# lukasino1214/soc_real_time_renderer

Hardware: AMD Instinct MI355X
Metric: frames/sec + ms/pass, Sponza 3840x2160 deferred+SSAO+TAA (higher is better)
Workload: dtype f32 (fp16/unorm8/d32 storage)

## Files before the change

include/soc_rt.h:

```cpp
#ifndef SOC_RT_H
#define SOC_RT_H

#include <stdint.h>
#include <stddef.h>

#ifdef __cplusplus
extern "C" {
#endif

#define SOC_RT_ABI_VERSION 1

#define SOC_OK 0
#define SOC_E_INVALID_ARG (-1)
#define SOC_E_SHAPE (-2)
#define SOC_E_HIP (-3)
#define SOC_E_UNSUPPORTED (-4)

struct ihipStream_t;
typedef struct ihipStream_t* soc_stream;

typedef enum soc_format {
    SOC_FMT_RGBA16F = 1,
    SOC_FMT_D32F = 2,
    SOC_FMT_R8_UNORM = 3,
// ... 240 lines not shown
#define SOC_PHASE_ALL 3

#define SOC_RENDERER_TIMING 1
#define SOC_RENDERER_UNFUSED_BLOOM 2
#define SOC_RENDERER_SERIAL 4
#define SOC_RENDERER_UNFUSED_TONEMAP 8
#define SOC_RENDERER_FUSED_HISTOGRAM 16
#define SOC_RENDERER_EXACT_BLOOM 32
#define SOC_RENDERER_UNFUSED_HISTOGRAM 64
#define SOC_RENDERER_NO_SKY_SPLIT 128
#define SOC_RENDERER_STATIC_INPUTS 256
#define SOC_RENDERER_VELOCITY_SLOTS 512
#define SOC_RENDERER_BLOOM_IN_COMPOSITION 1024
#define SOC_RENDERER_SKY_LANE_HIGH 2048
#define SOC_RENDERER_SKY_LANE_PROBE 4096

soc_renderer* soc_renderer_create(const soc_frame_images* images, uint32_t flags);
void soc_renderer_destroy(soc_renderer* r);
int soc_renderer_execute(soc_renderer* r, const soc_globals* g, int32_t phase, soc_stream stream);
int soc_renderer_set_exposure_pixels(soc_renderer* r, uint64_t total_pixels, int32_t wide_accumulator);
int32_t soc_renderer_pass_count(const soc_renderer* r);
const char* soc_renderer_pass_name(const soc_renderer* r, int32_t index);
const char* soc_renderer_pass_group(const soc_renderer* r, int32_t index);
float soc_renderer_pass_ms(soc_renderer* r, int32_t index);
#define SOC_RENDERER_TIMING_RING 256
int soc_renderer_set_pass_timing(soc_renderer* r, int32_t index, int32_t enable);
int soc_renderer_reset_timing(soc_renderer* r);
int soc_renderer_pass_stats(soc_renderer* r, int32_t index, float* total_ms, int32_t* frames);
int32_t soc_renderer_pass_event_times(soc_renderer* r, int32_t index, void* base, float* start_ms, float* end_ms,
                                      int32_t n);
int32_t soc_renderer_current_history(const soc_renderer* r);
int soc_renderer_set_current_history(soc_renderer* r, int32_t index);
int soc_renderer_set_async(soc_renderer* r, int32_t enable);
int32_t soc_renderer_side_queue(const soc_renderer* r);
int32_t soc_renderer_side_queue_probe_frames(const soc_renderer* r);

enum soc_resource {
    SOC_RES_ALBEDO = 0, SOC_RES_EMISSIVE, SOC_RES_NORMAL, SOC_RES_DEPTH, SOC_RES_VELOCITY,
    SOC_RES_SUN_SHADOW, SOC_RES_NOISE,
    SOC_RES_BLOOM_MIP0, SOC_RES_BLOOM_MIP1, SOC_RES_BLOOM_MIP2, SOC_RES_BLOOM_MIP3,
    SOC_RES_BLOOM_OUTPUT,
    SOC_RES_SSAO, SOC_RES_SSAO_BLUR, SOC_RES_CLOUDS, SOC_RES_COLOR,
    SOC_RES_PREVIOUS_COLOR, SOC_RES_RESOLVED,
    SOC_RES_PREVIOUS_VELOCITY,
    SOC_RES_AUTO_EXPOSURE,
    SOC_RES_OUTPUT,
    SOC_RES_VISIBILITY,
    SOC_RES_HISTOGRAM_PARTIALS,
    SOC_RES_SKY_COLOR,
    SOC_RES_SKY_HISTOGRAM_PARTIALS,
    SOC_RES_USER0 = 32,
    SOC_RES_COUNT = 64
};
#define SOC_PASS_MAX_USES 16
#define SOC_PASS_ASYNC 1
typedef struct soc_pass_desc {
    const char* name;
    const char* group;
    int32_t phase;
    uint32_t flags;
    int32_t read_count, write_count;
    int32_t reads[SOC_PASS_MAX_USES];
    int32_t writes[SOC_PASS_MAX_USES];
} soc_pass_desc;
typedef int32_t (*soc_pass_callback)(void* user, const soc_globals* g, const soc_frame_images* images, soc_stream stream);
int soc_renderer_add_pass(soc_renderer* r, const soc_pass_desc* desc, soc_pass_callback fn, void* user,
// ... 85 lines not shown
```

soc_real_time_renderer_amd/__init__.py:

```python
from __future__ import annotations

import ctypes as C
import os
from typing import Optional

import numpy as np
import torch

from . import _abi
from ._abi import (FMT_D32F, FMT_R8_UNORM, FMT_RGBA8_SRGB, FMT_RGBA8_UNORM, FMT_RGBA16F, FMT_RGBA32F,
                   PHASE_ALL, PHASE_POST_EXPOSURE, PHASE_PRE_EXPOSURE, AutoExposure, Camera, FrameImages, Globals,
                   SocImg)

PKG_DIR = os.path.dirname(os.path.abspath(__file__))
LIB_PATH = os.path.join(PKG_DIR, "lib", os.environ.get("SOC_RT_LIB_VARIANT", "libsoc_rt.so"))

__all__ = ["SocError", "lib", "img", "Globals", "Camera", "AutoExposure", "globals_defaults", "frame_update",
           "bloom_downsample", "bloom_upsample", "bloom_chain", "ssao_prepare_noise", "ssao_generation",
           "ssao_blur", "cloud_rendering", "composition", "generate_luminance_histogram",
           "resolve_luminance_histogram", "temporal_antialiasing", "copy_image", "tone_mapping", "upload_globals",
           "Renderer", "read_image", "write_png", "write_exr", "FMT_RGBA16F", "FMT_D32F", "FMT_R8_UNORM", "FMT_RGBA8_UNORM", "FMT_RGBA8_SRGB",
           "FMT_RGBA32F", "PHASE_PRE_EXPOSURE", "PHASE_POST_EXPOSURE", "PHASE_ALL"]


# ... 419 lines not shown
        _check(lib().soc_renderer_add_pass(self.handle, C.byref(d), cb, None, before.encode() if before else None),
               "soc_renderer_add_pass")
        self._callbacks = getattr(self, "_callbacks", []) + [cb]

    def pass_uses(self, index: int):
        rd, wr = C.c_uint64(0), C.c_uint64(0)
        _check(lib().soc_renderer_pass_uses(self.handle, index, C.byref(rd), C.byref(wr)), "soc_renderer_pass_uses")

        def names(m):
            return {(_abi.RESOURCES[b] if b < len(_abi.RESOURCES) else f"USER{b - _abi.RES_USER0}")
                    for b in range(_abi.RES_COUNT) if (m >> b) & 1}
        return names(rd.value), names(wr.value)

    def pass_dependencies(self, index: int):
        buf = (C.c_int32 * 64)()
        n = lib().soc_renderer_pass_dependencies(self.handle, index, buf, 64)
        if n < 0:
            _check(int(n), "soc_renderer_pass_dependencies")
        return [int(buf[i]) for i in range(min(n, 64))]

    def pass_carry_dependencies(self, index: int):
        buf = (C.c_int32 * 64)()
        n = lib().soc_renderer_pass_carry_dependencies(self.handle, index, buf, 64)
        if n < 0:
            _check(int(n), "soc_renderer_pass_carry_dependencies")
        return [int(buf[k]) for k in range(n)]

    def pass_lane(self, index: int) -> int:
        return int(lib().soc_renderer_pass_lane(self.handle, index))

    def set_async(self, enable: bool) -> None:
        _check(lib().soc_renderer_set_async(self.handle, int(bool(enable))), "soc_renderer_set_async")

    def current_history(self) -> int:
        return int(lib().soc_renderer_current_history(self.handle))

    def velocity_slot(self) -> int:
        return 1 - self.current_history()

    def resolved(self) -> torch.Tensor:
        return self.frame["history_color"][self.current_history()]

    STATE_VERSION = 1

    def save_state(self, path: Optional[str] = None) -> dict:
        torch.cuda.synchronize()
        h = self.current_history()
        st = {"version": np.int32(self.STATE_VERSION), "history_index": np.int32(h),
              "history_color": self.frame["history_color"][h].cpu().numpy(),
              "history_velocity": self.frame["history_velocity"][h].cpu().numpy(),
              "auto_exposure": self.frame["auto_exposure"].cpu().numpy()}
        if path:
            np.savez(path, **st)
        return st

    def load_state(self, state) -> None:
        st = dict(np.load(state, allow_pickle=False)) if isinstance(state, (str, os.PathLike)) else state
        if int(st["version"]) != self.STATE_VERSION:
            raise ValueError(f"load_state: checkpoint version {int(st['version'])}, expected {self.STATE_VERSION}")
        h = int(st["history_index"])
        if h not in (0, 1):
            raise ValueError(f"load_state: history_index {h} is not 0 or 1")
        srcs = {}
        for key in ("history_color", "history_velocity"):
            dst = self.frame[key][h]
            src = np.asarray(st[key])
# ... 24 lines not shown
```

soc_real_time_renderer_amd/_abi.py:

```python
from __future__ import annotations

import ctypes as C

SOC_OK = 0
SOC_E_INVALID_ARG = -1
SOC_E_SHAPE = -2
SOC_E_HIP = -3
SOC_E_UNSUPPORTED = -4

FMT_RGBA16F = 1
FMT_D32F = 2
FMT_R8_UNORM = 3
FMT_RGBA8_UNORM = 4
FMT_RGBA8_SRGB = 5
FMT_RGBA32F = 6

BYTES_PER_PIXEL = {FMT_RGBA16F: 8, FMT_D32F: 4, FMT_R8_UNORM: 1, FMT_RGBA8_UNORM: 4, FMT_RGBA8_SRGB: 4,
                   FMT_RGBA32F: 16}

MAX_POINT_LIGHTS = 128
MAX_SPOT_LIGHTS = 128
BIN_COUNT = 256
SSAO_MAX_KERNEL = 26

# ... 166 lines not shown
    "soc_mat4_ortho_rh_no": (None, [C.POINTER(C.c_float)] + [C.c_float] * 6),
    "soc_mat4_look_at_rh": (None, [C.POINTER(C.c_float)] * 4),
    "soc_mat4_inverse": (None, [C.POINTER(C.c_float)] * 2),
    "soc_mat4_mul": (None, [C.POINTER(C.c_float)] * 3),
    "soc_bloom_downsample": (_I, [_G, _IMG, _IMG, _P]),
    "soc_bloom_upsample": (_I, [_G, _IMG, _IMG, _P]),
    "soc_bloom_chain": (_I, [_G, _IMG, C.POINTER(SocImg), C.c_int32, _P]),
    "soc_bloom_weighted_stage": (_I, [_G, _IMG, C.POINTER(SocImg), C.c_int32, _IMG, C.c_int32, _P]),
    "soc_ssao_prepare_noise": (_I, [_IMG, _IMG, _P, _P]),
    "soc_ssao_generation": (_I, [_G, _IMG, _IMG, _IMG, _P, _P]),
    "soc_ssao_blur": (_I, [_G, _IMG, _IMG, _P]),
    "soc_cloud_rendering_workspace_size": (C.c_size_t, [C.c_int32, C.c_int32]),
    "soc_cloud_rendering": (_I, [_G, _IMG, _IMG, _IMG, _P, _P]),
    "soc_composition_luminance_histogram": (_I, [_G, _P, _IMG, _IMG, _IMG, _IMG, _IMG, _IMG, _IMG, _IMG, _P, _P, _P]),
    "soc_composition": (_I, [_G, _P, _IMG, _IMG, _IMG, _IMG, _IMG, _IMG, _IMG, _IMG, _P]),
    "soc_generate_luminance_histogram": (_I, [_G, _IMG, _P, _P]),
    "soc_resolve_luminance_histogram": (_I, [_G, _P, C.c_uint64, C.c_int32, _P]),
    "soc_temporal_antialiasing_tone_mapping": (_I, [_G, _IMG, _IMG, _IMG, _IMG, _IMG, _IMG, _IMG, _P, _IMG, _P]),
    "soc_temporal_antialiasing": (_I, [_G, _IMG, _IMG, _IMG, _IMG, _IMG, _IMG, _IMG, _P]),
    "soc_copy_image": (_I, [_IMG, _IMG, _P]),
    "soc_tone_mapping": (_I, [_G, _IMG, _P, _IMG, _P]),
    "soc_upload_globals": (_I, [_G, _P, _P]),
    "soc_renderer_create": (_P, [C.POINTER(FrameImages), C.c_uint32]),
    "soc_renderer_destroy": (None, [_P]),
    "soc_renderer_execute": (_I, [_P, _G, C.c_int32, _P]),
    "soc_renderer_set_exposure_pixels": (_I, [_P, C.c_uint64, C.c_int32]),
    "soc_renderer_pass_count": (C.c_int32, [_P]),
    "soc_renderer_pass_name": (C.c_char_p, [_P, C.c_int32]),
    "soc_renderer_pass_group": (C.c_char_p, [_P, C.c_int32]),
    "soc_renderer_pass_ms": (C.c_float, [_P, C.c_int32]),
    "soc_renderer_current_history": (C.c_int32, [_P]),
    "soc_renderer_set_current_history": (C.c_int, [_P, C.c_int32]),
    "soc_renderer_set_async": (C.c_int, [_P, C.c_int32]),
    "soc_scene_update": (_I, [C.POINTER(Globals), C.POINTER(Entity), C.c_int32, C.POINTER(C.c_float),
                              C.POINTER(C.c_float)]),
    "soc_renderer_add_pass": (_I, [_P, C.POINTER(PassDesc), PASS_CALLBACK, _P, C.c_char_p]),
    "soc_renderer_pass_uses": (_I, [_P, C.c_int32, C.POINTER(C.c_uint64), C.POINTER(C.c_uint64)]),
    "soc_renderer_pass_dependencies": (C.c_int32, [_P, C.c_int32, C.POINTER(C.c_int32), C.c_int32]),
    "soc_renderer_pass_carry_dependencies": (C.c_int32, [_P, C.c_int32, C.POINTER(C.c_int32), C.c_int32]),
    "soc_renderer_pass_lane": (C.c_int32, [_P, C.c_int32]),
    "soc_renderer_set_pass_timing": (_I, [_P, C.c_int32, C.c_int32]),
    "soc_renderer_reset_timing": (_I, [_P]),
    "soc_renderer_pass_stats": (_I, [_P, C.c_int32, C.POINTER(C.c_float), C.POINTER(C.c_int32)]),
    "soc_renderer_pass_event_times": (C.c_int32, [_P, C.c_int32, _P, C.POINTER(C.c_float), C.POINTER(C.c_float),
                                                  C.c_int32]),
    "soc_renderer_side_queue": (C.c_int32, [_P]),
    "soc_renderer_side_queue_probe_frames": (C.c_int32, [_P]),
    "soc_raster_workspace_size": (C.c_size_t, [C.c_int32, C.c_int32]),
    "soc_paired_texels_bytes": (C.c_size_t, [C.c_int32, C.c_int32]),
    "soc_renderer_set_raster_scene": (_I, [_P, C.POINTER(RasterScene)]),
    "soc_height_to_normal": (_I, [_IMG, _IMG, _P]),
    "soc_terrain_tess_counts": (_I, [_I, _I, C.POINTER(C.c_int32), C.POINTER(C.c_int32)]),
    "soc_terrain_tessellate": (_I, [_G, _IMG, _I, _I, _P, _P, _P, _P, _P]),
    "soc_mip_level_count": (_I, [_I, _I]),
    "soc_mip_chain_bytes": (C.c_size_t, [_I, _I, _I]),
    "soc_generate_mips": (_I, [_IMG, _P]),
    "soc_pair_textures": (_I, [_IMG, _IMG, _P, _P]),
    "soc_generate_hiz": (_I, [_G, _IMG, C.POINTER(SocImg), C.c_int32, C.c_int32, _P, _P]),
    "soc_renderer_metrics_json": (C.c_int64, [_P, C.c_uint64, C.c_char_p, C.c_size_t]),
    "soc_read_image": (_I, [_IMG, _P, C.c_int32, _P]),
    "soc_write_png": (_I, [C.c_char_p, _P, C.c_int32, C.c_int32, C.c_int32]),
    "soc_write_exr": (_I, [C.c_char_p, _P, C.c_int32, C.c_int32, C.c_int32]),
    "soc_raster_visibility": (_I, [C.POINTER(Mesh), C.POINTER(C.c_float), C.c_int32, _P, C.c_int32, C.c_int32,
                                   C.c_int32, _P, _P]),
    "soc_raster_depth": (_I, [C.POINTER(Mesh), C.POINTER(C.c_float), C.c_int32, C.c_float, C.c_float, _IMG, _P, _P]),
    "soc_gbuffer_resolve": (_I, [_G, C.POINTER(Mesh), _P, C.c_int32, _P, _IMG, _IMG, _IMG, _IMG, _IMG, _P, _P]),
# ... 13 lines not shown
```

soc_real_time_renderer_amd/csrc/capi.cpp:

```cpp
#include <hip/hip_runtime.h>

#include <cmath>
#include <cstdarg>
#include <cstdlib>
#include <cstdio>
#include <cstring>
#include <functional>
#include <string>
#include <mutex>
#include <vector>

#include "soc_internal.hpp"

namespace soc {

static thread_local std::string t_error;

int set_error(int code, const char* fmt, ...) {
    char buf[512];
    va_list ap;
    va_start(ap, fmt);
    vsnprintf(buf, sizeof buf, fmt, ap);
    va_end(ap);
    t_error = buf;
// ... 574 lines not shown
        soc_pass_callback fn;
        void* user;
    };
    soc_frame_images img{};
    soc_raster_scene scene{};
    bool has_scene = false;
    std::vector<Pass> passes;
    std::vector<UserPass> user_passes;
    uint32_t flags = 0;
    int hist = 0;
    uint64_t total_pixels = 0;
    int wide = 0;
    soc_globals* staging = nullptr;
    hipEvent_t staging_ev[4] = {nullptr, nullptr, nullptr, nullptr};
    int staging_slot = 0;
    bool async = true;
    int side_device = -1;
    hipStream_t side = nullptr;
    hipEvent_t fork_ev = nullptr, join_ev = nullptr;
    hipStream_t lane_q[2] = {nullptr, nullptr};
    int side_queue = -1;
    int probe_frames = 0;
    hipEvent_t probe_ev[16] = {};
    hipEvent_t switch_ev = nullptr;
    uint32_t* hist_scratch = nullptr;
    void* shadow_ws = nullptr;
    size_t shadow_ws_bytes = 0;
    bool fold_in_resolve = false;
    bool sky_split = false, sky_split_active = false;
    bool bloom_in_comp = false;
    bool bloom_in_comp_ok = false;
    bool main_after_side = true;
    bool inputs_ordered = false;
};

namespace {
using PassFn = soc_renderer::PassFn;

uint64_t res_mask(std::initializer_list<int> ids) {
    uint64_t m = 0;
    for (int i : ids) m |= 1ull << i;
    return m;
}

uint64_t widen_velocity(const soc_renderer* r, uint64_t m) {
    const uint64_t both = (1ull << SOC_RES_VELOCITY) | (1ull << SOC_RES_PREVIOUS_VELOCITY);
    return (r->flags & SOC_RENDERER_VELOCITY_SLOTS) && (m & both) ? m | both : m;
}

soc_img frame_velocity(const soc_renderer* r) {
    return (r->flags & SOC_RENDERER_VELOCITY_SLOTS) ? r->img.history_velocity[1 - r->hist] : r->img.velocity;
}

bool sky_lane_high(const soc_renderer* r) {
    return r->side_queue == 1 || (r->side_queue == -1 && r->lane_q[0] && r->side == r->lane_q[0]);
}
bool bloom_in_comp_active(const soc_renderer* r) {
    return r->bloom_in_comp && r->bloom_in_comp_ok && (sky_lane_high(r) || tuning_knob("SOC_RENDERER_BLOOM_IN_COMP_ANY_LANE", 0));
}

soc_renderer::Pass& add_pass(soc_renderer* r, std::string name, std::string group, int phase, uint64_t reads,
                             uint64_t writes, PassFn fn, uint32_t flags = 0) {
    soc_renderer::Pass p;
    p.name = std::move(name);
    p.group = std::move(group);
    p.phase = phase;
// ... 85 lines not shown
                     return soc_bloom_upsample(g, r->img.bloom_mips[i], r->img.bloom_mips[i - 1], (soc_stream)s);
                 });
    add_pass(r, "BloomUpsample - 0", "Bloom", pre, res_mask({mip[0]}), res_mask({dst_res}),
             [r](const soc_globals* g, hipStream_t s) {
                 const soc_img& dst = r->img.bloom_output.data ? r->img.bloom_output : r->img.emissive;
                 return soc_bloom_upsample(g, r->img.bloom_mips[0], dst, (soc_stream)s);
             });
}

void build_passes_tail(soc_renderer* r) {
    auto& I = r->img;
    const int pre = SOC_PHASE_PRE_EXPOSURE, post = SOC_PHASE_POST_EXPOSURE;
    const int em_res = I.bloom_output.data ? SOC_RES_BLOOM_OUTPUT : SOC_RES_EMISSIVE;
    add_pass(r, "SSAOGeneration", "Ambient Occlusion", pre, res_mask({SOC_RES_DEPTH, SOC_RES_NORMAL}),
             res_mask({SOC_RES_SSAO}), [r](const soc_globals* g, hipStream_t s) {
                 return soc_ssao_generation(g, r->img.depth, r->img.normal, r->img.ssao, r->img.ssao_noise_table,
                                            (soc_stream)s);
             });
    add_pass(r, "SSAOBlur", "Ambient Occlusion", pre, res_mask({SOC_RES_SSAO}), res_mask({SOC_RES_SSAO_BLUR}),
             [r](const soc_globals* g, hipStream_t s) { return soc_ssao_blur(g, r->img.ssao, r->img.ssao_blur, (soc_stream)s); });
    const bool fused_hist = !(r->flags & SOC_RENDERER_UNFUSED_HISTOGRAM);
    const soc_img& em_img = I.bloom_output.data ? I.bloom_output : I.emissive;
    soc_globals gres{};
    gres.resolution[0] = I.color.width;
    gres.resolution[1] = I.color.height;
    r->sky_split = fused_hist && !(r->flags & SOC_RENDERER_NO_SKY_SPLIT) &&
                   soc::composition_pair_applicable(&gres, I.color, I.albedo, em_img, I.normal, I.depth, I.clouds);
    const uint64_t sky_w = r->sky_split ? res_mask({SOC_RES_SKY_COLOR, SOC_RES_SKY_HISTOGRAM_PARTIALS}) : 0;
    const uint64_t parts = res_mask({SOC_RES_HISTOGRAM_PARTIALS}) | (r->sky_split ? res_mask({SOC_RES_SKY_HISTOGRAM_PARTIALS}) : 0);
    add_pass(r, "CloudRendering", "Sky Rendering", pre, res_mask({SOC_RES_DEPTH, SOC_RES_NOISE}), res_mask({SOC_RES_CLOUDS}),
             [r](const soc_globals* g, hipStream_t s) {
                 const bool sky_bound = sky_lane_high(r) && tuning_knob("SOC_RENDERER_SKY_BOUND_VARIANTS", 1);
                 return soc::cloud_rendering_launch(g, r->img.depth, r->img.noise, r->img.clouds, r->img.clouds_workspace,
                                                    (soc_stream)s, sky_bound);
             }, SOC_PASS_ASYNC);
    if (r->sky_split)
        add_pass(r, "SkyCompose", "Sky Rendering", pre, res_mask({SOC_RES_CLOUDS, SOC_RES_DEPTH}), sky_w,
                 [r](const soc_globals* g, hipStream_t s) {
                     return soc::sky_compose_launch(g, r->img.color, r->img.depth, r->img.clouds, r->hist_scratch,
                                                    (soc_stream)s);
                 }, SOC_PASS_ASYNC);
    const uint64_t comp_reads = res_mask({SOC_RES_ALBEDO, em_res, SOC_RES_NORMAL, SOC_RES_DEPTH, SOC_RES_SSAO_BLUR,
                                          SOC_RES_SUN_SHADOW}) | (r->bloom_in_comp ? res_mask({SOC_RES_BLOOM_MIP1}) : 0) |
                                (r->sky_split ? 0 : res_mask({SOC_RES_CLOUDS}));
    if (fused_hist) {
        add_pass(r, "Composition+GenerateLuminanceHistogram", "Composition", pre, comp_reads,
                 res_mask({SOC_RES_COLOR, SOC_RES_HISTOGRAM_PARTIALS}), [r](const soc_globals* g, hipStream_t s) {
                     const auto& I = r->img;
                     const soc_img& em = I.bloom_output.data ? I.bloom_output : I.emissive;
                     return soc::composition_luminance_histogram(g, I.d_globals, I.color, I.albedo, em, I.normal, I.depth,
                                                                 I.ssao_blur, I.shadow, I.clouds, I.auto_exposure,
                                                                 r->hist_scratch, false, (soc_stream)s,
                                                                 r->sky_split_active,
                                                                 bloom_in_comp_active(r) ? &I.bloom_mips[1] : nullptr);
                 });
        auto& fold = add_pass(r, "LuminanceHistogramFold", "Auto Exposure", pre, parts,
                              res_mask({SOC_RES_AUTO_EXPOSURE}) | parts,
                              [r](const soc_globals* g, hipStream_t s) {
                                  (void)g;
                                  return soc::histogram_fold_launch(r->hist_scratch, r->img.auto_exposure, (soc_stream)s);
                              });
        fold.skip = [r] { return r->fold_in_resolve; };
    } else {
        add_pass(r, "Composition", "Composition", pre, comp_reads, res_mask({SOC_RES_COLOR}),
                 [r](const soc_globals* g, hipStream_t s) {
                     const auto& I = r->img;
                     const soc_img& em = I.bloom_output.data ? I.bloom_output : I.emissive;
// ... 248 lines not shown
    int rc = p.run(g, s);
    if (rc) return rc;
    if (p.timed) {
        (void)hipEventRecord(p.ev1[slot], s);
        p.last = slot;
        p.next = (slot + 1) % SOC_RENDERER_TIMING_RING;
        if (p.count < SOC_RENDERER_TIMING_RING) p.count++;
    }
    return SOC_OK;
}

static void destroy_side_lane(soc_renderer* r) {
    for (hipEvent_t* e : {&r->fork_ev, &r->join_ev, &r->switch_ev})
        if (*e) { (void)hipEventDestroy(*e); *e = nullptr; }
    for (auto& e : r->probe_ev)
        if (e) { (void)hipEventDestroy(e); e = nullptr; }
    if (r->lane_q[0] || r->lane_q[1]) {
        for (auto& q : r->lane_q)
            if (q) { (void)hipStreamDestroy(q); q = nullptr; }
    } else if (r->side) {
        (void)hipStreamDestroy(r->side);
    }
    r->side = nullptr;
    r->side_queue = -1;
    r->probe_frames = 0;
}

static int ensure_side_lane(soc_renderer* r) {
    int dev = 0;
    if (hipGetDevice(&dev) != hipSuccess) return set_error(SOC_E_HIP, "soc_renderer_execute: hipGetDevice failed");
    if (r->side && r->side_device == dev) return SOC_OK;
    if (r->side) {
        destroy_side_lane(r);
        for (auto& p : r->passes)
            if (p.done) { (void)hipEventDestroy(p.done); p.done = nullptr; p.done_recorded = false; }
    }
    const int sq_flags = (r->flags & SOC_RENDERER_SKY_LANE_HIGH) ? 1 : (r->flags & SOC_RENDERER_SKY_LANE_PROBE) ? 3 : 2;
    int sq = tuning_knob("SOC_RENDERER_SIDE_QUEUE", sq_flags);
    int least = 0, greatest = 0;
    if (hipDeviceGetStreamPriorityRange(&least, &greatest) != hipSuccess || least == greatest) sq = 0;
    hipError_t se = hipSuccess;
    if (sq == 3) {
        se = hipStreamCreateWithPriority(&r->lane_q[0], hipStreamNonBlocking, greatest);
        if (se == hipSuccess) se = hipStreamCreateWithPriority(&r->lane_q[1], hipStreamNonBlocking, least);
        if (se == hipSuccess) se = hipEventCreateWithFlags(&r->switch_ev, device_event_flags());
        for (auto& e : r->probe_ev)
            if (se == hipSuccess) se = hipEventCreate(&e);
        r->side = r->lane_q[0];
        r->side_queue = -1;
        r->probe_frames = 0;
    } else if (const int cus = tuning_knob("SOC_RENDERER_SKY_CUS", 0); cus > 0 && cus < 32) {
        int dev_cus = 256;
        (void)hipDeviceGetAttribute(&dev_cus, hipDeviceAttributeMultiprocessorCount, dev);
        const int layout = tuning_knob("SOC_RENDERER_SKY_CU_LAYOUT", 0);
        std::vector<uint32_t> mask((size_t)(dev_cus + 31) / 32, 0u);
        for (int i = 0; i < dev_cus; ++i)
            if ((layout ? i % 32 : (i / 8) % 32) < cus) mask[(size_t)i / 32] |= 1u << (i % 32);
        se = hipExtStreamCreateWithCUMask(&r->side, (uint32_t)mask.size(), mask.data());
        r->side_queue = 0;
    } else if (sq == 1 || sq == 2) {
        se = hipStreamCreateWithPriority(&r->side, hipStreamNonBlocking, sq == 2 ? least : greatest);
        r->side_queue = sq;
    } else {
        se = hipStreamCreateWithFlags(&r->side, hipStreamNonBlocking);
        r->side_queue = 0;
    }
// ... 284 lines not shown
}

extern "C" int soc_renderer_pass_uses(const soc_renderer* r, int32_t i, uint64_t* reads, uint64_t* writes) {
    if (!r || i < 0 || i >= (int32_t)r->passes.size() || !reads || !writes)
        return set_error(SOC_E_INVALID_ARG, "soc_renderer_pass_uses: bad arguments");
    *reads = r->passes[i].reads;
    *writes = r->passes[i].writes;
    return SOC_OK;
}

extern "C" int32_t soc_renderer_pass_dependencies(const soc_renderer* r, int32_t i, int32_t* out, int32_t cap) {
    if (!r || i < 0 || i >= (int32_t)r->passes.size() || cap < 0 || (cap > 0 && !out))
        return set_error(SOC_E_INVALID_ARG, "soc_renderer_pass_dependencies: bad arguments");
    const auto& d = r->passes[i].deps;
    for (int k = 0; k < (int)d.size() && k < cap; ++k) out[k] = d[k];
    return (int32_t)d.size();
}

extern "C" int32_t soc_renderer_pass_carry_dependencies(const soc_renderer* r, int32_t i, int32_t* out, int32_t cap) {
    if (!r || i < 0 || i >= (int32_t)r->passes.size() || cap < 0 || (cap > 0 && !out))
        return set_error(SOC_E_INVALID_ARG, "soc_renderer_pass_carry_dependencies: bad arguments");
    const auto& d = r->passes[i].carry;
    for (int k = 0; k < (int)d.size() && k < cap; ++k) out[k] = d[k];
    return (int32_t)d.size();
}

extern "C" int32_t soc_renderer_pass_lane(const soc_renderer* r, int32_t i) {
    if (!r || i < 0 || i >= (int32_t)r->passes.size()) return set_error(SOC_E_INVALID_ARG, "soc_renderer_pass_lane: bad index");
    return (r->passes[i].flags & SOC_PASS_ASYNC) ? 1 : 0;
}

extern "C" int soc_renderer_set_async(soc_renderer* r, int32_t enable) {
    if (!r) return set_error(SOC_E_INVALID_ARG, "soc_renderer_set_async: null renderer");
    r->async = enable != 0;
    return SOC_OK;
}

extern "C" int soc_renderer_set_exposure_pixels(soc_renderer* r, uint64_t total_pixels, int32_t wide_accumulator) {
    if (!r) return set_error(SOC_E_INVALID_ARG, "soc_renderer_set_exposure_pixels: null renderer");
    r->total_pixels = total_pixels;
    r->wide = wide_accumulator;
    return SOC_OK;
}

extern "C" int32_t soc_renderer_pass_count(const soc_renderer* r) { return r ? (int32_t)r->passes.size() : 0; }

extern "C" const char* soc_renderer_pass_name(const soc_renderer* r, int32_t i) {
    if (!r || i < 0 || i >= (int32_t)r->passes.size()) return nullptr;
    return r->passes[i].name.c_str();
}

extern "C" const char* soc_renderer_pass_group(const soc_renderer* r, int32_t i) {
    if (!r || i < 0 || i >= (int32_t)r->passes.size()) return nullptr;
    return r->passes[i].group.c_str();
}

extern "C" float soc_renderer_pass_ms(soc_renderer* r, int32_t i) {
    if (!r || i < 0 || i >= (int32_t)r->passes.size()) return -1.0f;
    auto& p = r->passes[i];
    if (!p.timed || p.last < 0) return -1.0f;
    float ms = -1.0f;
    if (hipEventElapsedTime(&ms, p.ev0[p.last], p.ev1[p.last]) != hipSuccess) return -1.0f;
    return ms;
}

extern "C" int64_t soc_renderer_metrics_json(soc_renderer* r, uint64_t frame, char* buf, size_t cap) {
    if (!r) return set_error(SOC_E_INVALID_ARG, "soc_renderer_metrics_json: null renderer");
// ... 106 lines not shown
```

soc_real_time_renderer_amd/csrc/clouds.hip:

```cpp
#include <cstdlib>
#include <type_traits>

#include "soc_internal.hpp"

#ifndef SOC_CLOUDS_EXITS
#define SOC_CLOUDS_EXITS 1
#endif
#ifndef SOC_CLOUDS_PROFILE
#define SOC_CLOUDS_PROFILE 0
#endif

namespace soc {
namespace {

#ifndef SOC_CLOUDS_PRECISE
#define SOC_CLOUDS_PRECISE 0
#endif
#ifndef SOC_CLOUDS_EXACT
#define SOC_CLOUDS_EXACT 1
#endif
__device__ __forceinline__ float cl_exp(float x) {
    if constexpr (SOC_CLOUDS_PRECISE != 0) return expf(x);
    else return __expf(x);
}
__device__ __forceinline__ float cl_exp2(float x) {
    if constexpr (SOC_CLOUDS_PRECISE != 0) return exp2f(x);
    else return __builtin_amdgcn_exp2f(x);
}
__device__ __forceinline__ float cl_sqrt(float x) {
    if constexpr (SOC_CLOUDS_PRECISE != 0) return sqrtf(x);
    else return __builtin_amdgcn_sqrtf(x);
}
__device__ __forceinline__ float cl_log2(float x) {
// ... 666 lines not shown
        if (k3 < N16) d = src[k3];
        dst[k0] = a;
        if (k1 < N16) dst[k1] = b;
        if (k2 < N16) dst[k2] = c;
        if (k3 < N16) dst[k3] = d;
    }
}

__device__ __forceinline__ bool is_sky(const CloudParams& p, const DImg& depth, int x, int y) {
    return sample_f32(depth, div_rn((float)x, p.res_x_m1, p.r_res_x_m1), div_rn((float)y, p.res_y_m1, p.r_res_y_m1)) ==
           1.0f;
}

template <bool NOISE_R8>
__global__ __launch_bounds__(kWorkgroup) void clouds_kernel(DImg depth, DImg noise, DImg target, CloudParams p) {
    __shared__ uint32_t quads[kTable];
    const int x = blockIdx.x * TX + threadIdx.x, y = blockIdx.y * TY + threadIdx.y;
    const int tid = threadIdx.y * TX + threadIdx.x;
    const bool inside = x < p.res_x && y < p.res_y && x < target.w && y < target.h;
    const bool sky = inside && is_sky(p, depth, x, y);
    if (!__syncthreads_or(sky)) {
        if (inside) row_ptr_w<uint32_t>(target, y)[x] = pack_unorm8x4(f4{0.2f, 0.4f, 1.0f, 1.0f});
        return;
    }
    stage_noise<NOISE_R8>(noise, quads, tid, TX * TY);
    __syncthreads();
    if (!inside) return;
    row_ptr_w<uint32_t>(target, y)[x] = sky ? shade_sky(p, quads, x, y) : pack_unorm8x4(f4{0.2f, 0.4f, 1.0f, 1.0f});
}

constexpr int kClassifyTiles = 4;
template <bool HOIST>
__global__ __launch_bounds__(kWorkgroup) void clouds_classify(DImg depth, DImg target, CloudParams p, int vec_store,
                                                       uint32_t* __restrict__ counter, uint32_t* __restrict__ list) {
    __shared__ uint32_t wave_total[kClassifyTiles][4];
    __shared__ uint32_t wg_base;
    const int lane = threadIdx.x & 63, wave = threadIdx.x >> 6;
    const int x0 = blockIdx.x * 64 + (wave & 1) * 32 + (lane & 7) * 4;
    const int W = min(p.res_x, target.w), H = min(p.res_y, target.h);
    const uint32_t other = pack_unorm8x4(f4{0.2f, 0.4f, 1.0f, 1.0f});
    const unsigned long long below = (1ull << lane) - 1ull;
    uint32_t masks = 0;
    uint32_t before[kClassifyTiles];
    float dk[kClassifyTiles][4];
    auto load_all = [&](auto sample) {
#pragma unroll
        for (int k = 0; k < kClassifyTiles; ++k) {
            const int y = min((blockIdx.y * kClassifyTiles + k) * 16 + (wave >> 1) * 8 + (lane >> 3), H - 1);
            const float ray_v = div_rn((float)y, p.res_y_m1, p.r_res_y_m1);
#pragma unroll
            for (int j = 0; j < 4; ++j) dk[k][j] = sample(div_rn((float)min(x0 + j, W - 1), p.res_x_m1, p.r_res_x_m1), ray_v);
        }
    };
    if (HOIST && depth.w >= 2) {
        load_all([&](float u, float v) {
            const Axis ax = axis_clamp(u, depth.w), ay = axis_clamp(v, depth.h);
            typedef float f2u4 __attribute__((ext_vector_type(2))) __attribute__((aligned(4)));
            const f2u4 r0 = *reinterpret_cast<const f2u4*>(row_ptr<float>(depth, ay.i0) + ax.i0);
            const f2u4 r1 = *reinterpret_cast<const f2u4*>(row_ptr<float>(depth, ay.i1) + ax.i0);
            return bilerp1(r0.x, r0.y, r1.x, r1.y, ax.w, ay.w);
        });
    } else if (HOIST) {
        load_all([&](float u, float v) { return sample_f32(depth, u, v); });
    }
#pragma unroll
    for (int k = 0; k < kClassifyTiles; ++k) {
        const int y = (blockIdx.y * kClassifyTiles + k) * 16 + (wave >> 1) * 8 + (lane >> 3);
        uint32_t mask = 0;
        if (y < H) {
// ... 409 lines not shown
            row_ptr_w<uint32_t>(target, y)[x] = pack_unorm8x4(f4{color.x, color.y, color.z, 1.0f});
        }
        __syncthreads();
    }
}

template <typename K>
int resident_blocks(K kernel, int threads = 256) {
    int dev = 0, cus = 256, per_cu = 0;
    (void)hipGetDevice(&dev);
    hipDeviceProp_t prop;
    if (hipGetDeviceProperties(&prop, dev) == hipSuccess && prop.multiProcessorCount > 0) cus = prop.multiProcessorCount;
    if (hipOccupancyMaxActiveBlocksPerMultiprocessor(&per_cu, kernel, threads, 0) != hipSuccess || per_cu < 1) per_cu = 2;
    return per_cu * cus;
}

}
}

using namespace soc;

namespace {
constexpr size_t kDensityBlocks = 3072;
struct CloudWs {
    uint32_t* counter;
    uint32_t* list;
    float4* atmos;
    PairBufs pb;
    float2* od_lut;
    uint32_t* noise_quads;
    uint2* noise_wide;
    uint32_t* noise_rows;
    float4* sky_tab;
    size_t bytes;
};
CloudWs cloud_ws_layout(void* base, size_t n) {
    auto al = [](size_t v) { return (v + 255) & ~(size_t)255; };
    char* b = static_cast<char*>(base);
    CloudWs w;
    size_t off = 256;
    w.counter = reinterpret_cast<uint32_t*>(b);
    w.list = reinterpret_cast<uint32_t*>(b + off);
    off = al(off + n * 4);
    w.atmos = reinterpret_cast<float4*>(b + off);
    off = al(off + n * 16);
    w.pb.counts = w.counter + 8;
    w.pb.pix_mask = reinterpret_cast<uint32_t*>(b + off);
    off = al(off + n * 4);
    w.pb.batch_base = reinterpret_cast<uint32_t*>(b + off);
    off = al(off + (n / 256 + 1) * 4);
    w.pb.geom = reinterpret_cast<float4*>(b + off);
    off = al(off + n * 32);
    w.pb.cap = (uint32_t)((2 * n + kShards - 1) / kShards);
    w.pb.pairs = reinterpret_cast<uint32_t*>(b + off);
    off = al(off + (size_t)kShards * w.pb.cap * 4);
    w.pb.od = reinterpret_cast<float*>(b + off);
    off = al(off + (size_t)kShards * w.pb.cap * 4);
    w.pb.vis = reinterpret_cast<float*>(b + off);
    off = al(off + (size_t)kShards * w.pb.cap * 4);
    w.pb.od_tmp = reinterpret_cast<float*>(b + off);
    w.pb.od_blocks = (uint32_t)std::min<size_t>(kDensityBlocks, (n + 255) / 256);
    w.pb.n = (uint32_t)n;
    off = al(off + (size_t)w.pb.od_blocks * 24 * 256 * 4);
    w.od_lut = reinterpret_cast<float2*>(b + off);
    off = al(off + (size_t)kOdR * kOdM * sizeof(float2));
    w.sky_tab = reinterpret_cast<float4*>(b + off);
    off = al(off + (size_t)kSvEntries * 2 * sizeof(float4));
    w.noise_quads = reinterpret_cast<uint32_t*>(b + off);
    off = al(off + (size_t)kTableU32 * 4);
    w.noise_wide = reinterpret_cast<uint2*>(b + off);
    off = al(off + (size_t)kTableU2 * 8);
    w.noise_rows = reinterpret_cast<uint32_t*>(b + off);
    off = al(off + (size_t)kRowU32 * 4);
    w.bytes = off;
    return w;
}
}

extern "C" size_t soc_cloud_rendering_workspace_size(int32_t width, int32_t height) {
    if (width <= 0 || height <= 0) return 0;
    return cloud_ws_layout(nullptr, (size_t)width * (size_t)height).bytes;
}

extern "C" int soc_cloud_rendering(const soc_globals* g, soc_img depth, soc_img noise, soc_img target, void* workspace,
                                   soc_stream stream) {
    return soc::cloud_rendering_launch(g, depth, noise, target, workspace, stream, false);
}

int soc::cloud_rendering_launch(const soc_globals* g, soc_img depth, soc_img noise, soc_img target, void* workspace,
                                soc_stream stream, bool sky_bound) {
    static const char* P = "soc_cloud_rendering";
    if (!g) return set_error(SOC_E_INVALID_ARG, "%s: null globals", P);
    int rc = check_img(depth, SOC_FMT_D32F, P, "depth");
    if (!rc) rc = check_img(target, SOC_FMT_RGBA8_UNORM, P, "target");
    if (!rc) rc = check_img(noise, 0, P, "noise");
    if (rc) return rc;
    if (noise.format != SOC_FMT_R8_UNORM && noise.format != SOC_FMT_RGBA8_UNORM)
        return set_error(SOC_E_UNSUPPORTED, "%s: noise must be R8_UNORM or RGBA8_UNORM", P);
    if (noise.width != 64 || noise.height != 64)
        return set_error(SOC_E_SHAPE, "%s: noise texture must be 64x64 (assets/Clouds/noise.png)", P);
    CloudParams p;
    p.inv_proj = mat4(g->camera_inverse_projection_matrix);
    p.inv_view = mat4(g->camera_inverse_view_matrix);
    for (int i = 0; i < 3; ++i) {
        p.sun[i] = -g->sun_info.direction[i];
        p.cam[i] = g->camera_position[i];
    }
    p.res_x = g->resolution[0];
    p.res_y = g->resolution[1];
    p.res_x_m1 = (float)g->resolution[0] - 1.0f;
    p.res_y_m1 = (float)g->resolution[1] - 1.0f;
    p.r_res_x_m1 = recip_rn(g->resolution[0] - 1);
    p.r_res_y_m1 = recip_rn(g->resolution[1] - 1);
    p.elapsed = g->elapsed_time;
    p.sun_factor = fmaxf(fminf(fabsf(p.sun[0]), fabsf(p.sun[2])) + p.sun[1], 0.0f);
    const int W = std::min(target.width, p.res_x), H = std::min(target.height, p.res_y);
    if (W <= 0 || H <= 0) return SOC_OK;
    if (W > 65535 || H > 65535) return set_error(SOC_E_SHAPE, "%s: extent above 65535", P);
    hipStream_t s = hs(stream);
    const bool r8 = noise.format == SOC_FMT_R8_UNORM;
    if (!workspace) {
        dim3 blk(TX, TY), grd(ceil_div(W, TX), ceil_div(H, TY));
        if (r8) launch("clouds_kernel", kWorkgroup, clouds_kernel<true>, grd, blk, 0, s, dimg(depth), dimg(noise), dimg(target), p);
        else launch("clouds_kernel", kWorkgroup, clouds_kernel<false>, grd, blk, 0, s, dimg(depth), dimg(noise), dimg(target), p);
        return check_launch("cloud_rendering");
    }
    CloudWs ws = cloud_ws_layout(workspace, (size_t)target.width * (size_t)target.height);
    ws.pb.store_geom = (uint32_t)tuning_knob("SOC_CLOUDS_GEOM", 1);
    uint32_t* counter = ws.counter;
    uint32_t* list = ws.list;
    OdLut lut{nullptr, 0.0f};
    const bool use_lut = SOC_CLOUDS_PROFILE < 4 && tuning_knob("SOC_CLOUDS_OD_LUT", 1);
    const bool noise_tab = tuning_knob("SOC_CLOUDS_NOISE_TABLE", 1) != 0;
    const float C2 = p.sun[0] * p.sun[0] + p.sun[1] * p.sun[1] + p.sun[2] * p.sun[2];
    if (use_lut) lut = OdLut{ws.od_lut, C2};
    ws.pb.noise_quads = noise_tab ? ws.noise_quads : nullptr;
    ws.pb.noise_wide = noise_tab ? ws.noise_wide : nullptr;
    ws.pb.noise_rows = noise_tab ? ws.noise_rows : nullptr;
    {
        const int lut_blocks = use_lut ? ceil_div(kOdR * kOdM, kWorkgroup) : 1;
        const int blocks_all = lut_blocks + (noise_tab ? ceil_div(kTableBuild, kWorkgroup) : 0);
        float2* lt = use_lut ? ws.od_lut : nullptr;
        if (noise.format == SOC_FMT_R8_UNORM)
            launch("clouds_od_lut", kWorkgroup, clouds_od_lut<true>, blocks_all, kWorkgroup, 0, s, lt, C2, counter, lut_blocks,
                   dimg(noise), ws.noise_quads, ws.noise_wide, ws.noise_rows);
        else
            launch("clouds_od_lut", kWorkgroup, clouds_od_lut<false>, blocks_all, kWorkgroup, 0, s, lt, C2, counter, lut_blocks,
                   dimg(noise), ws.noise_quads, ws.noise_wide, ws.noise_rows);
    }
    const int vec_store = (target.pitch_bytes % 16 == 0) && (reinterpret_cast<uintptr_t>(target.data) % 16 == 0);
    const bool hoist = sky_bound || tuning_knob("SOC_CLOUDS_CLASSIFY_HOIST", 0);
    if (hoist)
        launch("clouds_classify", kWorkgroup, clouds_classify<true>, dim3(ceil_div(W, 64), ceil_div(H, 16 * kClassifyTiles)),
               kWorkgroup, 0, s, dimg(depth), dimg(target), p, vec_store, counter, list);
    else
        launch("clouds_classify", kWorkgroup, clouds_classify<false>, dim3(ceil_div(W, 64), ceil_div(H, 16 * kClassifyTiles)),
               kWorkgroup, 0, s, dimg(depth), dimg(target), p, vec_store, counter, list);
    static int res_atmos = 0, res_density = 0, res_sunvis = 0, res_sunvis_n = 0, res_sunvis_r = 0, res_resolve = 0;
    if (!res_atmos) {
        res_atmos = resident_blocks(clouds_atmosphere<false>);
        res_density = resident_blocks(clouds_density<false>);
        res_sunvis = resident_blocks(clouds_sunvis<false, kSunvisLanes, true>, kSunvisLanes);
        res_sunvis_n = resident_blocks(clouds_sunvis<false, kSunvisLanes, false, true>, kSunvisLanes);
        res_sunvis_r = resident_blocks(clouds_sunvis<false, kSunvisLanes, false, true, true>, kSunvisLanes);
        res_resolve = resident_blocks(clouds_resolve<false, true>);
    }
    const long long blocks = ((long long)W * H + 255) / 256;
    if (SOC_CLOUDS_PROFILE >= 4) return check_launch("cloud_rendering");
    const int gmul = std::max(1, tuning_knob("SOC_CLOUDS_GRID_MULT", 2));
    auto grid = [&](int res, long long items_blocks) { return (int)std::max(1LL, std::min<long long>(res, items_blocks)); };
    auto grid_m = [&](int res, long long items_blocks) {
        return (int)std::max(1LL, std::min<long long>((long long)res * gmul, items_blocks));
    };
    const int apos_knob = tuning_knob("SOC_CLOUDS_ATMOS_POS", -1);
    const int apos = apos_knob >= 0 ? apos_knob : ((long long)W * H > 2560LL * 1440LL ? 2 : 0);
    SkyTab st{};
    st.t = nullptr;
    if (lut.t && tuning_knob("SOC_CLOUDS_SKY_TABLE", 1)) {
        const double r0x = (double)(0.0f + p.cam[0]), r0y = (double)(6372e3f + p.cam[1]), r0z = (double)(0.0f + p.cam[2]);
        const double rl = std::sqrt(r0x * r0x + r0y * r0y + r0z * r0z);
        const double ux = r0x / rl, uy = r0y / rl, uz = r0z / rl;
        const double sx = p.sun[0], sy = p.sun[1], sz = p.sun[2], su = sx * ux + sy * uy + sz * uz;
        double hx = sx - su * ux, hy = sy - su * uy, hz = sz - su * uz, hl = std::sqrt(hx * hx + hy * hy + hz * hz);
        if (!(hl > 1e-9)) {
            hx = uy; hy = -ux; hz = 0.0;
            hl = std::sqrt(hx * hx + hy * hy);
            if (!(hl > 1e-9)) { hx = 1.0; hy = 0.0; hz = 0.0; hl = 1.0; }
        }
        hx /= hl; hy /= hl; hz /= hl;
        const double bx = uy * hz - uz * hy, by = uz * hx - ux * hz, bz = ux * hy - uy * hx;
// ... 45 lines not shown
        else if (!sv_wide)
            launch("clouds_sunvis", kSunvisLanes, clouds_sunvis<true, kSunvisLanes, false, true>, grid_m(res_sunvis_n, blocks), kSunvisLanes, 0, s, nz, p, list, ws.pb);
        else if (sv_pf)
            launch("clouds_sunvis", kSunvisLanes, clouds_sunvis<true, kSunvisLanes, true, true>, grid_m(res_sunvis, blocks), kSunvisLanes, 0, s, nz, p, list, ws.pb);
        else
            launch("clouds_sunvis", kSunvisLanes, clouds_sunvis<true, kSunvisLanes, true>, grid_m(res_sunvis, blocks), kSunvisLanes, 0, s, nz, p, list, ws.pb);
        if (apos == 2) atmos();
        if (fold && rb == 4) resolve(clouds_resolve<true, true, 4>);
        else if (fold && rb == 8) resolve(clouds_resolve<true, true, 8>);
        else if (fold) resolve(clouds_resolve<true, true>);
        else resolve(clouds_resolve<true, false>);
    } else {
        if (drows) launch("clouds_density", kWorkgroup, clouds_density<false, 8, true>, density_grid, kWorkgroup, 0, s, nz, p, counter, list, ws.pb);
        else if (db == 4) launch("clouds_density", kWorkgroup, clouds_density<false, 4>, density_grid, kWorkgroup, 0, s, nz, p, counter, list, ws.pb);
        else if (db == 8) launch("clouds_density", kWorkgroup, clouds_density<false, 8>, density_grid, kWorkgroup, 0, s, nz, p, counter, list, ws.pb);
        else launch("clouds_density", kWorkgroup, clouds_density<false>, density_grid, kWorkgroup, 0, s, nz, p, counter, list, ws.pb);
        if (apos == 1) atmos();
        if (sv_table == 2)
            launch("clouds_sunvis", kSunvisLanes, clouds_sunvis<false, kSunvisLanes, false, true, true>, grid_m(res_sunvis_r, blocks), kSunvisLanes, 0, s, nz, p, list, ws.pb);
        else if (!sv_wide)
            launch("clouds_sunvis", kSunvisLanes, clouds_sunvis<false, kSunvisLanes, false, true>, grid_m(res_sunvis_n, blocks), kSunvisLanes, 0, s, nz, p, list, ws.pb);
        else if (sv_pf)
            launch("clouds_sunvis", kSunvisLanes, clouds_sunvis<false, kSunvisLanes, true, true>, grid_m(res_sunvis, blocks), kSunvisLanes, 0, s, nz, p, list, ws.pb);
        else
            launch("clouds_sunvis", kSunvisLanes, clouds_sunvis<false, kSunvisLanes, true>, grid_m(res_sunvis, blocks), kSunvisLanes, 0, s, nz, p, list, ws.pb);
        if (apos == 2) atmos();
        if (fold && rb == 4) resolve(clouds_resolve<false, true, 4>);
        else if (fold && rb == 8) resolve(clouds_resolve<false, true, 8>);
        else if (fold) resolve(clouds_resolve<false, true>);
        else resolve(clouds_resolve<false, false>);
    }
    return check_launch("cloud_rendering");
}
```

soc_real_time_renderer_amd/csrc/soc_internal.hpp:

```cpp
#pragma once

#include <hip/hip_runtime.h>
#include <stdint.h>

#include <cstdarg>
#include <cstdio>
#include <string>

#include "../../include/soc_rt.h"
#include "soc_device.hpp"

namespace soc {

int set_error(int code, const char* fmt, ...);
void clear_error();

inline int bytes_per_pixel(int fmt) {
    switch (fmt) {
    case SOC_FMT_RGBA16F: return 8;
    case SOC_FMT_D32F: return 4;
    case SOC_FMT_R8_UNORM: return 1;
    case SOC_FMT_RGBA8_UNORM:
    case SOC_FMT_RGBA8_SRGB: return 4;
    case SOC_FMT_RGBA32F: return 16;
// ... 18 lines not shown

inline hipStream_t hs(soc_stream s) { return reinterpret_cast<hipStream_t>(s); }

int tuning_knob(const char* name, int dflt);
inline float recip_rn(int n) {
    return n >= 1 && n <= 16384 ? 1.0f / (float)n : 0.0f;
}

int check_launch(const char* pass);

bool block_fits(const char* kernel, int bound, dim3 block);
template <typename... P, typename... A>
inline void launch(const char* kernel, int bound, void (*k)(P...), dim3 grid, dim3 block, size_t lds, hipStream_t s,
                   A&&... args) {
    if (!block_fits(kernel, bound, block)) return;
    k<<<grid, block, lds, s>>>(static_cast<P>(args)...);
}

inline unsigned ceil_div(unsigned a, unsigned b) { return (a + b - 1) / b; }

void agx_matrices(float compression, float M[9], float Minv[9]);
void mat4_mul_host(float out[16], const float a[16], const float b[16]);

bool bloom_fused_applicable(const soc_img& emissive, const soc_img* mips, int mip_count, const soc_img& output);
int launch_bloom_weighted(const soc_img& emissive, const soc_img* mips, const soc_img& output, hipStream_t s, int stage);

int composition_luminance_histogram(const soc_globals* g, const soc_globals* d_globals, soc_img target, soc_img albedo,
                                    soc_img emissive, soc_img normal, soc_img depth, soc_img ssao, soc_img shadow,
                                    soc_img clouds, soc_auto_exposure* ae, uint32_t* scratch, bool fold, soc_stream stream,
                                    bool sky_external = false, const soc_img* bloom_mip1 = nullptr);
bool composition_pair_applicable(const soc_globals* g, const soc_img& target, const soc_img& albedo,
                                 const soc_img& emissive, const soc_img& normal, const soc_img& depth,
                                 const soc_img& clouds);
int cloud_rendering_launch(const soc_globals* g, soc_img depth, soc_img noise, soc_img target, void* workspace,
                           soc_stream stream, bool sky_bound);
int sky_compose_launch(const soc_globals* g, soc_img target, soc_img depth, soc_img clouds, uint32_t* scratch,
                       soc_stream stream);
int histogram_fold_launch(uint32_t* scratch, soc_auto_exposure* ae, soc_stream stream);
int resolve_luminance_histogram(const soc_globals* g, soc_auto_exposure* ae, uint64_t total_pixels, int32_t wide_accumulator,
                                uint32_t* scratch, soc_stream stream);

}
```

Before: 1864.

## Cache cloud OD LUT and noise tables across frames; ping-pong classify counters

Adds a per-renderer CloudState that tracks whether the optical-depth LUT and noise tables are still valid, keyed on the C2 constant and the noise image pointer, format and pitch. Rebuilds of these tables are skipped when nothing changed. The classify counter block now alternates between two buffers, and each frame's classify kernel zeroes the buffer the next frame will use, so the per-frame clear folds into existing work. The caching is disabled for sky-bound runs above 1440p unless a knob overrides it. The risk is stale tables if the noise contents change under the same pointer, so an explicit invalidate API is exposed.

```diff
diff --git a/include/soc_rt.h b/include/soc_rt.h
--- a/include/soc_rt.h
+++ b/include/soc_rt.h
@@ -296,6 +296,7 @@
 int32_t soc_renderer_current_history(const soc_renderer* r);
 int soc_renderer_set_current_history(soc_renderer* r, int32_t index);
 int soc_renderer_set_async(soc_renderer* r, int32_t enable);
+int soc_renderer_invalidate_cloud_tables(soc_renderer* r);
 int32_t soc_renderer_side_queue(const soc_renderer* r);
 int32_t soc_renderer_side_queue_probe_frames(const soc_renderer* r);
 
diff --git a/soc_real_time_renderer_amd/__init__.py b/soc_real_time_renderer_amd/__init__.py
--- a/soc_real_time_renderer_amd/__init__.py
+++ b/soc_real_time_renderer_amd/__init__.py
@@ -475,6 +475,9 @@
     def set_async(self, enable: bool) -> None:
         _check(lib().soc_renderer_set_async(self.handle, int(bool(enable))), "soc_renderer_set_async")
 
+    def invalidate_cloud_tables(self) -> None:
+        _check(lib().soc_renderer_invalidate_cloud_tables(self.handle), "soc_renderer_invalidate_cloud_tables")
+
     def current_history(self) -> int:
         return int(lib().soc_renderer_current_history(self.handle))
 
diff --git a/soc_real_time_renderer_amd/_abi.py b/soc_real_time_renderer_amd/_abi.py
--- a/soc_real_time_renderer_amd/_abi.py
+++ b/soc_real_time_renderer_amd/_abi.py
@@ -222,6 +222,7 @@
     "soc_renderer_current_history": (C.c_int32, [_P]),
     "soc_renderer_set_current_history": (C.c_int, [_P, C.c_int32]),
     "soc_renderer_set_async": (C.c_int, [_P, C.c_int32]),
+    "soc_renderer_invalidate_cloud_tables": (C.c_int, [_P]),
     "soc_scene_update": (_I, [C.POINTER(Globals), C.POINTER(Entity), C.c_int32, C.POINTER(C.c_float),
                               C.POINTER(C.c_float)]),
     "soc_renderer_add_pass": (_I, [_P, C.POINTER(PassDesc), PASS_CALLBACK, _P, C.c_char_p]),
diff --git a/soc_real_time_renderer_amd/csrc/capi.cpp b/soc_real_time_renderer_amd/csrc/capi.cpp
--- a/soc_real_time_renderer_amd/csrc/capi.cpp
+++ b/soc_real_time_renderer_amd/csrc/capi.cpp
@@ -630,6 +630,7 @@
     bool bloom_in_comp_ok = false;
     bool main_after_side = true;
     bool inputs_ordered = false;
+    soc::CloudState clouds_state;
 };
 
 namespace {
@@ -781,7 +782,7 @@
              [r](const soc_globals* g, hipStream_t s) {
                  const bool sky_bound = sky_lane_high(r) && tuning_knob("SOC_RENDERER_SKY_BOUND_VARIANTS", 1);
                  return soc::cloud_rendering_launch(g, r->img.depth, r->img.noise, r->img.clouds, r->img.clouds_workspace,
-                                                    (soc_stream)s, sky_bound);
+                                                    (soc_stream)s, sky_bound, &r->clouds_state);
              }, SOC_PASS_ASYNC);
     if (r->sky_split)
         add_pass(r, "SkyCompose", "Sky Rendering", pre, res_mask({SOC_RES_CLOUDS, SOC_RES_DEPTH}), sky_w,
@@ -1096,6 +1097,7 @@
     if (r->side && r->side_device == dev) return SOC_OK;
     if (r->side) {
         destroy_side_lane(r);
+        r->clouds_state.reset();
         for (auto& p : r->passes)
             if (p.done) { (void)hipEventDestroy(p.done); p.done = nullptr; p.done_recorded = false; }
     }
@@ -1446,7 +1448,16 @@
 
 extern "C" int soc_renderer_set_async(soc_renderer* r, int32_t enable) {
     if (!r) return set_error(SOC_E_INVALID_ARG, "soc_renderer_set_async: null renderer");
+    if (r->async != (enable != 0)) {
+        r->inputs_ordered = false;
+    }
     r->async = enable != 0;
+    return SOC_OK;
+}
+
+extern "C" int soc_renderer_invalidate_cloud_tables(soc_renderer* r) {
+    if (!r) return set_error(SOC_E_INVALID_ARG, "soc_renderer_invalidate_cloud_tables: null renderer");
+    r->clouds_state.reset();
     return SOC_OK;
 }
 
diff --git a/soc_real_time_renderer_amd/csrc/clouds.hip b/soc_real_time_renderer_amd/csrc/clouds.hip
--- a/soc_real_time_renderer_amd/csrc/clouds.hip
+++ b/soc_real_time_renderer_amd/csrc/clouds.hip
@@ -1,4 +1,5 @@
 #include <cstdlib>
+#include <cstring>
 #include <type_traits>
 
 #include "soc_internal.hpp"
@@ -731,9 +732,11 @@
 constexpr int kClassifyTiles = 4;
 template <bool HOIST>
 __global__ __launch_bounds__(kWorkgroup) void clouds_classify(DImg depth, DImg target, CloudParams p, int vec_store,
-                                                       uint32_t* __restrict__ counter, uint32_t* __restrict__ list) {
+                                                       uint32_t* __restrict__ counter, uint32_t* __restrict__ list,
+                                                       uint32_t* __restrict__ zero_next) {
     __shared__ uint32_t wave_total[kClassifyTiles][4];
     __shared__ uint32_t wg_base;
+    if (zero_next && (blockIdx.x | blockIdx.y) == 0 && threadIdx.x < 64) zero_next[threadIdx.x] = 0u;
     const int lane = threadIdx.x & 63, wave = threadIdx.x >> 6;
     const int x0 = blockIdx.x * 64 + (wave & 1) * 32 + (lane & 7) * 4;
     const int W = min(p.res_x, target.w), H = min(p.res_y, target.h);
@@ -1209,6 +1212,7 @@
     uint2* noise_wide;
     uint32_t* noise_rows;
     float4* sky_tab;
+    uint32_t* counter_b;
     size_t bytes;
 };
 CloudWs cloud_ws_layout(void* base, size_t n) {
@@ -1249,6 +1253,8 @@
     off = al(off + (size_t)kTableU2 * 8);
     w.noise_rows = reinterpret_cast<uint32_t*>(b + off);
     off = al(off + (size_t)kRowU32 * 4);
+    w.counter_b = reinterpret_cast<uint32_t*>(b + off);
+    off += 256;
     w.bytes = off;
     return w;
 }
@@ -1264,8 +1270,23 @@
     return soc::cloud_rendering_launch(g, depth, noise, target, workspace, stream, false);
 }
 
+namespace {
+int cloud_rendering_queue(const soc_globals* g, soc_img depth, soc_img noise, soc_img target, void* workspace,
+                          soc_stream stream, bool sky_bound, CloudState* state);
+}
 int soc::cloud_rendering_launch(const soc_globals* g, soc_img depth, soc_img noise, soc_img target, void* workspace,
-                                soc_stream stream, bool sky_bound) {
+                                soc_stream stream, bool sky_bound, CloudState* state) {
+    const int rc = cloud_rendering_queue(g, depth, noise, target, workspace, stream, sky_bound, state);
+    if (rc && state) {
+        state->blocks_primed = false;
+        state->invalidate_tables();
+    }
+    return rc;
+}
+
+namespace {
+int cloud_rendering_queue(const soc_globals* g, soc_img depth, soc_img noise, soc_img target, void* workspace,
+                          soc_stream stream, bool sky_bound, CloudState* state) {
     static const char* P = "soc_cloud_rendering";
     if (!g) return set_error(SOC_E_INVALID_ARG, "%s: null globals", P);
     int rc = check_img(depth, SOC_FMT_D32F, P, "depth");
@@ -1304,7 +1325,6 @@
     }
     CloudWs ws = cloud_ws_layout(workspace, (size_t)target.width * (size_t)target.height);
     ws.pb.store_geom = (uint32_t)tuning_knob("SOC_CLOUDS_GEOM", 1);
-    uint32_t* counter = ws.counter;
     uint32_t* list = ws.list;
     OdLut lut{nullptr, 0.0f};
     const bool use_lut = SOC_CLOUDS_PROFILE < 4 && tuning_knob("SOC_CLOUDS_OD_LUT", 1);
@@ -1314,10 +1334,54 @@
     ws.pb.noise_quads = noise_tab ? ws.noise_quads : nullptr;
     ws.pb.noise_wide = noise_tab ? ws.noise_wide : nullptr;
     ws.pb.noise_rows = noise_tab ? ws.noise_rows : nullptr;
-    {
-        const int lut_blocks = use_lut ? ceil_div(kOdR * kOdM, kWorkgroup) : 1;
-        const int blocks_all = lut_blocks + (noise_tab ? ceil_div(kTableBuild, kWorkgroup) : 0);
-        float2* lt = use_lut ? ws.od_lut : nullptr;
+    const int static_knob = tuning_knob("SOC_CLOUDS_STATIC_TABLES", -1);
+    const bool static_tables = static_knob >= 0 ? static_knob != 0 : !(sky_bound && (long long)W * H > 2560LL * 1440LL);
+    const bool cached = state && SOC_CLOUDS_PROFILE < 4 && static_tables;
+    uint32_t* counter = ws.counter;
+    uint32_t* zero_next = nullptr;
+    bool build_od = use_lut, build_noise = noise_tab;
+    if (cached) {
+        if (state->workspace != workspace) {
+            state->invalidate_tables();
+            state->blocks_primed = false;
+            state->workspace = workspace;
+        }
+        if (!state->blocks_primed) {
+            if (hipMemsetAsync(ws.counter, 0, 256, s) != hipSuccess || hipMemsetAsync(ws.counter_b, 0, 256, s) != hipSuccess)
+                return set_error(SOC_E_HIP, "%s: counter block clear failed", P);
+            state->blocks_primed = true;
+        }
+        uint32_t c2_bits;
+        memcpy(&c2_bits, &C2, sizeof c2_bits);
+        if (state->od_valid && state->c2_bits != c2_bits) state->od_valid = false;
+        if (state->noise_valid && (state->noise_data != noise.data || state->noise_format != noise.format ||
+                                   state->noise_pitch != noise.pitch_bytes))
+            state->noise_valid = false;
+        build_od = use_lut && !state->od_valid;
+        build_noise = noise_tab && !state->noise_valid;
+        if (build_od) {
+            state->od_valid = true;
+            state->c2_bits = c2_bits;
+        }
+        if (build_noise) {
+            state->noise_valid = true;
+            state->noise_data = noise.data;
+            state->noise_format = noise.format;
+            state->noise_pitch = noise.pitch_bytes;
+        }
+        counter = (state->frame & 1u) ? ws.counter_b : ws.counter;
+        zero_next = (state->frame & 1u) ? ws.counter : ws.counter_b;
+        state->frame++;
+    } else if (state) {
+        state->invalidate_tables();
+        state->blocks_primed = false;
+        state->workspace = nullptr;
+    }
+    ws.pb.counts = counter + 8;
+    if (!cached || build_od || build_noise) {
+        const int lut_blocks = build_od ? ceil_div(kOdR * kOdM, kWorkgroup) : 1;
+        const int blocks_all = lut_blocks + (build_noise ? ceil_div(kTableBuild, kWorkgroup) : 0);
+        float2* lt = build_od ? ws.od_lut : nullptr;
         if (noise.format == SOC_FMT_R8_UNORM)
             launch("clouds_od_lut", kWorkgroup, clouds_od_lut<true>, blocks_all, kWorkgroup, 0, s, lt, C2, counter, lut_blocks,
                    dimg(noise), ws.noise_quads, ws.noise_wide, ws.noise_rows);
@@ -1329,10 +1393,10 @@
     const bool hoist = sky_bound || tuning_knob("SOC_CLOUDS_CLASSIFY_HOIST", 0);
     if (hoist)
         launch("clouds_classify", kWorkgroup, clouds_classify<true>, dim3(ceil_div(W, 64), ceil_div(H, 16 * kClassifyTiles)),
-               kWorkgroup, 0, s, dimg(depth), dimg(target), p, vec_store, counter, list);
+               kWorkgroup, 0, s, dimg(depth), dimg(target), p, vec_store, counter, list, zero_next);
     else
         launch("clouds_classify", kWorkgroup, clouds_classify<false>, dim3(ceil_div(W, 64), ceil_div(H, 16 * kClassifyTiles)),
-               kWorkgroup, 0, s, dimg(depth), dimg(target), p, vec_store, counter, list);
+               kWorkgroup, 0, s, dimg(depth), dimg(target), p, vec_store, counter, list, zero_next);
     static int res_atmos = 0, res_density = 0, res_sunvis = 0, res_sunvis_n = 0, res_sunvis_r = 0, res_resolve = 0;
     if (!res_atmos) {
         res_atmos = resident_blocks(clouds_atmosphere<false>);
@@ -1444,3 +1508,4 @@
     }
     return check_launch("cloud_rendering");
 }
+}
diff --git a/soc_real_time_renderer_amd/csrc/soc_internal.hpp b/soc_real_time_renderer_amd/csrc/soc_internal.hpp
--- a/soc_real_time_renderer_amd/csrc/soc_internal.hpp
+++ b/soc_real_time_renderer_amd/csrc/soc_internal.hpp
@@ -74,8 +74,19 @@
 bool composition_pair_applicable(const soc_globals* g, const soc_img& target, const soc_img& albedo,
                                  const soc_img& emissive, const soc_img& normal, const soc_img& depth,
                                  const soc_img& clouds);
+struct CloudState {
+    bool od_valid = false, noise_valid = false;
+    uint32_t c2_bits = 0;
+    const void* noise_data = nullptr;
+    int32_t noise_format = 0, noise_pitch = 0;
+    void* workspace = nullptr;
+    bool blocks_primed = false;
+    uint32_t frame = 0;
+    void invalidate_tables() { od_valid = noise_valid = false; }
+    void reset() { *this = CloudState(); }
+};
 int cloud_rendering_launch(const soc_globals* g, soc_img depth, soc_img noise, soc_img target, void* workspace,
-                           soc_stream stream, bool sky_bound);
+                           soc_stream stream, bool sky_bound, CloudState* state = nullptr);
 int sky_compose_launch(const soc_globals* g, soc_img target, soc_img depth, soc_img clouds, uint32_t* scratch,
                        soc_stream stream);
 int histogram_fold_launch(uint32_t* scratch, soc_auto_exposure* ae, soc_stream stream);
```

Result: faster. 1883, median of 6 (+1.0%).
